# abdel-habib/mmg-clip

Hardware: AMD Instinct MI355X
Metric: image-text pairs/sec (global batch) (higher is better)
Workload: dtype bf16; 1 GPU; C2: train_binary_class_clf, ConvNeXt-tiny 1024x1024x1 + BERT-base S=77, LinearProjection 768->512, CLIPLoss, AdamW, all parameters trained; global_batch=256, per_gpu_batch=256, micro_batch=256, streams=text tower on a side stream, parallelism=dp1, loss_scope=local, text_dropout=HF training-mode dropout live (hidden 0.1, atte…

## Files before the change

### mmg-clip_amd/csrc/cnblock_mlp.hip

```cpp
#include "common.h"
#include <stdlib.h>


struct MlpFwd {
    const bf16_t* xd;
    const float* ln_w; const float* ln_b; float eps;
    const bf16_t* wt;
    const float* b1; const float* b2; const float* gamma;
    const bf16_t* res;
    bf16_t* y;
    bf16_t* hpre;
    bf16_t* xln;
    float* mean; float* rstd;
    long M; int ntiles;
    int nt;
    bf16_t* gact;
    int hkind;
};

__device__ __forceinline__ void mlp_glds16(const void* gsrc, void* lds_wave_base) {
    __builtin_amdgcn_global_load_lds((const __attribute__((address_space(1))) void*)gsrc,
                                     (__attribute__((address_space(3))) void*)lds_wave_base, 16, 0, 0);
}

template <int C> struct MlpCfg {
    static constexpr int NC = (C <= 128) ? 64 : 32;
    static constexpr int MT = (C <= 256) ? 2 : 1;
    static constexpr int WAVES = (C <= 256) ? 4 : 8;
    static constexpr int THREADS = WAVES * 64;
    static constexpr int BM = WAVES * 16 * MT;
    static constexpr int WGS = (C <= 96) ? 3 : (C <= 192 ? 2 : 1);
    static constexpr int WGS_BWD = (C <= 192) ? 2 : 1;
};

struct PackPart { const float* src; int w2_like; const float* scale; int btype; };
struct PackArgs { PackPart part[3]; int parts; bf16_t* out; int C, NC; };

__global__ __launch_bounds__(256) void mlp_pack_kernel(const PackArgs a) {
    const int C = a.C, NC = a.NC, H4 = 4 * C;
    const long per_part = (long)NC * C, per_chunk = per_part * a.parts, total = per_chunk * (H4 / NC);
    for (long e = (long)blockIdx.x * blockDim.x + threadIdx.x; e < total; e += (long)gridDim.x * blockDim.x) {
        const int j = (int)(e / per_chunk);
        long off = e - (long)j * per_chunk;
        const int pi = (int)(off / per_part);
        off -= (long)pi * per_part;
        const PackPart pp = a.part[pi];
        int n, c;
        if (!pp.btype) {
            const int kg = (int)(off / (NC * 8)), nn = (int)((off / 8) % NC), jj = (int)(off % 8);
            const int g32 = nn >> 5, tt = (nn >> 4) & 1, q = (nn >> 2) & 3, r = nn & 3;
            n = j * NC + 32 * g32 + 8 * q + 4 * tt + r; c = 8 * kg + jj;
        } else {
            const int kg = (int)(off / (C * 8)), jj = (int)(off % 8);
            const int cp = (int)((off / 8) % C);
            c = (cp & ~31) + 8 * ((cp >> 2) & 3) + 4 * ((cp >> 4) & 1) + (cp & 3);
            n = j * NC + 8 * kg + jj;
        }
        float v = pp.w2_like ? pp.src[(long)c * H4 + n] : pp.src[(long)n * C + c];
        if (pp.scale) v *= pp.scale[c];
        a.out[e] = f2bf(v);
    }
}

#ifdef MLP_PROBE
__device__ unsigned long long g_mlp_probe[8];
MMG_API int mmg_debug_mlp_probe(unsigned long long* out8, int reset) {
    if (out8 && hipMemcpyFromSymbol(out8, HIP_SYMBOL(g_mlp_probe), 64) != hipSuccess) return 1;
    unsigned long long z[8] = {0, 0, 0, 0, 0, 0, 0, 0};
    if (reset && hipMemcpyToSymbol(HIP_SYMBOL(g_mlp_probe), z, 64) != hipSuccess) return 1;
    return 0;
}
#define PROBE_T(var) const long long var = __builtin_readcyclecounter()
#define PROBE_ADD(acc, a, b) acc += (b) - (a)
#else
#define PROBE_T(var)
#define PROBE_ADD(acc, a, b)
#endif

template <int C, bool SAVE, int RW = 0>
__global__ __launch_bounds__(RW ? RW * 64 : MlpCfg<C>::THREADS, RW ? RW / 4 : MlpCfg<C>::WGS) void cnblock_mlp_fwd_kernel(const MlpFwd p) {
    constexpr bool RES = RW > 0;
    constexpr int NC = MlpCfg<C>::NC, MT = MlpCfg<C>::MT, MLP_THREADS = RES ? RW * 64 : MlpCfg<C>::THREADS;
    constexpr int MLP_BM = RES ? 16 * MT : MlpCfg<C>::BM;
    constexpr int KS1 = C / 32, CT = C / 16, NSUB = NC / 32, NCH = 4 * C / NC;
    constexpr int PART = NC * C * 2, CHUNK = 2 * PART, LOADS = CHUNK / 16 / MLP_THREADS;
    static_assert(CHUNK % (16 * MLP_THREADS) == 0, "chunk must be a whole number of 16-byte granules per thread");
    static_assert(NCH % 2 == 0, "ring parity is carried across tiles");
    static_assert(!RES || (!SAVE && NCH * CHUNK + 8 * C * 4 <= 160 * 1024), "resident form: every chunk image in LDS, nothing saved");
    extern __shared__ __attribute__((aligned(16))) char smem[];
    float* s_lnw = reinterpret_cast<float*>(smem + (RES ? NCH : 2) * CHUNK);
    float* s_lnb = s_lnw + C;
    float* s_b1 = s_lnb + C;
    float* s_b2 = s_b1 + 4 * C;
    float* s_gm = s_b2 + C;

    const int tid = threadIdx.x, lane = tid & 63;
    const int wave = RES ? __builtin_amdgcn_readfirstlane(tid >> 6) : tid >> 6;
    const int li = lane & 15, lg = lane >> 4;
    char* lds_wave = smem + (tid & ~63) * 16;
    const char* wsrc = reinterpret_cast<const char*>(p.wt) + tid * 16;

    auto stage = [&](int buf, int ch) {
        const char* s = wsrc + (size_t)ch * CHUNK;
#pragma unroll
        for (int it = 0; it < LOADS; ++it) mlp_glds16(s + it * (MLP_THREADS * 16), lds_wave + buf * CHUNK + it * (MLP_THREADS * 16));
    };
    if constexpr (RES) {
#pragma unroll
        for (int ch = 0; ch < NCH; ++ch) stage(ch, ch);
    } else if ((int)blockIdx.x < p.ntiles) stage(0, 0);
    for (int i = tid; i < C; i += MLP_THREADS) {
        s_lnw[i] = p.ln_w[i]; s_lnb[i] = p.ln_b[i]; s_b2[i] = p.b2[i]; s_gm[i] = p.gamma[i];
    }
    for (int i = tid; i < 4 * C; i += MLP_THREADS) s_b1[i] = p.b1[i];
    if constexpr (RES) asm volatile("s_waitcnt vmcnt(0)" ::: "memory");
    __syncthreads();

#ifdef MLP_PROBE
    long long pr_wait = 0, pr_g1 = 0, pr_gelu = 0, pr_g2 = 0;
#endif
    PROBE_T(pr_start);
    for (int tile = RES ? (int)blockIdx.x * RW + wave : (int)blockIdx.x; tile < p.ntiles; tile += RES ? (int)gridDim.x * RW : (int)gridDim.x) {
        const long row0 = RES ? (long)tile * MLP_BM + li : (long)tile * MLP_BM + wave * (16 * MT) + li;
        bf16x8 xf[MT][KS1];
#pragma unroll
        for (int mi = 0; mi < MT; ++mi) {
            const long row = row0 + 16 * mi;
            const long rr = row < p.M ? row : p.M - 1;
            uint4 raw[KS1];
#pragma unroll
            for (int ks = 0; ks < KS1; ++ks) raw[ks] = *reinterpret_cast<const uint4*>(p.xd + rr * C + 32 * ks + 8 * lg);
            float v[KS1][8];
            float s = 0.f;
#pragma unroll
            for (int ks = 0; ks < KS1; ++ks) {
                const unsigned w[4] = {raw[ks].x, raw[ks].y, raw[ks].z, raw[ks].w};
#pragma unroll
                for (int e = 0; e < 4; ++e) {
                    v[ks][2 * e] = bf2f_lo(w[e]); v[ks][2 * e + 1] = bf2f_hi(w[e]);
                    s += v[ks][2 * e] + v[ks][2 * e + 1];
                }
            }
            s += __shfl_xor(s, 16, 64); s += __shfl_xor(s, 32, 64);
            const float mean = s * (1.0f / C);
            float q = 0.f;
#pragma unroll
            for (int ks = 0; ks < KS1; ++ks)
#pragma unroll
                for (int e = 0; e < 8; ++e) { const float d = v[ks][e] - mean; q = fmaf(d, d, q); }
            q += __shfl_xor(q, 16, 64); q += __shfl_xor(q, 32, 64);
            const float rstd = rsqrtf(q * (1.0f / C) + p.eps);
            if (SAVE && lg == 0 && row < p.M) { p.mean[row] = mean; p.rstd[row] = rstd; }
#pragma unroll
            for (int ks = 0; ks < KS1; ++ks) {
                const f32x4 w0 = *reinterpret_cast<const f32x4*>(s_lnw + 32 * ks + 8 * lg);
                const f32x4 w1 = *reinterpret_cast<const f32x4*>(s_lnw + 32 * ks + 8 * lg + 4);
                const f32x4 c0 = *reinterpret_cast<const f32x4*>(s_lnb + 32 * ks + 8 * lg);
                const f32x4 c1 = *reinterpret_cast<const f32x4*>(s_lnb + 32 * ks + 8 * lg + 4);
                const float g[8] = {w0[0], w0[1], w0[2], w0[3], w1[0], w1[1], w1[2], w1[3]};
                const float b[8] = {c0[0], c0[1], c0[2], c0[3], c1[0], c1[1], c1[2], c1[3]};
                unsigned o[4];
#pragma unroll
                for (int e = 0; e < 4; ++e)
                    o[e] = pack2bf(fmaf((v[ks][2 * e] - mean) * rstd, g[2 * e], b[2 * e]),
                                   fmaf((v[ks][2 * e + 1] - mean) * rstd, g[2 * e + 1], b[2 * e + 1]));
                typedef __attribute__((ext_vector_type(4))) unsigned u32x4_t;
                xf[mi][ks] = __builtin_bit_cast(bf16x8, (u32x4_t{o[0], o[1], o[2], o[3]}));
                if (SAVE && p.xln && row < p.M) *reinterpret_cast<uint4*>(p.xln + row * C + 32 * ks + 8 * lg) = make_uint4(o[0], o[1], o[2], o[3]);
            }
        }

        f32x4 yacc[MT][CT];
#pragma unroll
        for (int mi = 0; mi < MT; ++mi)
#pragma unroll
            for (int ct = 0; ct < CT; ++ct) yacc[mi][ct] = f32x4{0.f, 0.f, 0.f, 0.f};

        for (int ch = 0; ch < NCH; ++ch) {
            PROBE_T(pr_a);
            if constexpr (!RES) {
                asm volatile("s_waitcnt vmcnt(0)" ::: "memory");
                __builtin_amdgcn_s_barrier();
            }
            PROBE_T(pr_b);
            PROBE_ADD(pr_wait, pr_a, pr_b);
            if constexpr (!RES) {
                if (ch + 1 < NCH) stage((ch + 1) & 1, ch + 1);
                else if (tile + (int)gridDim.x < p.ntiles) stage(0, 0);
            }
            const char* wb = smem + (RES ? ch : (ch & 1)) * CHUNK;
#pragma unroll
            for (int sub = 0; sub < NSUB; ++sub) {
#if defined(MLP_PROBE) && MLP_PROBE >= 2
                PROBE_T(pr_c);
#endif
                const int n0 = ch * NC + sub * 32 + 8 * lg;
                const f32x4 bia0 = *reinterpret_cast<const f32x4*>(s_b1 + n0);
                const f32x4 bia1 = *reinterpret_cast<const f32x4*>(s_b1 + n0 + 4);
                f32x4 hacc[MT][2];
#pragma unroll
                for (int mi = 0; mi < MT; ++mi) { hacc[mi][0] = bia0; hacc[mi][1] = bia1; }
#pragma unroll
                for (int ks = 0; ks < KS1; ++ks) {
#pragma unroll
                    for (int tt = 0; tt < 2; ++tt) {
                        const bf16x8 wf = *reinterpret_cast<const bf16x8*>(wb + (((4 * ks + lg) * NC + (2 * sub + tt) * 16 + li) << 4));
#pragma unroll
                        for (int mi = 0; mi < MT; ++mi)
                            hacc[mi][tt] = __builtin_amdgcn_mfma_f32_16x16x32_bf16(wf, xf[mi][ks], hacc[mi][tt], 0, 0, 0);
                    }
                }
#if defined(MLP_PROBE) && MLP_PROBE >= 2
                asm volatile("" : "+v"(hacc[0][0]), "+v"(hacc[MT - 1][1]));
                PROBE_T(pr_d);
                PROBE_ADD(pr_g1, pr_c, pr_d);
#endif
                bf16x8 gf[MT];
#pragma unroll
                for (int mi = 0; mi < MT; ++mi) {
                    const f32x4 h0 = hacc[mi][0], h1 = hacc[mi][1];
                    if (SAVE) {
                        const long row = row0 + 16 * mi;
                        if (row < p.M) {
                            if (p.hkind)
                                store16_stream(p.hpre + row * (4 * C) + n0,
                                               make_uint4(pack2bf(gelu_bf16_grad_poly(h0[0]), gelu_bf16_grad_poly(h0[1])), pack2bf(gelu_bf16_grad_poly(h0[2]), gelu_bf16_grad_poly(h0[3])),
                                                          pack2bf(gelu_bf16_grad_poly(h1[0]), gelu_bf16_grad_poly(h1[1])), pack2bf(gelu_bf16_grad_poly(h1[2]), gelu_bf16_grad_poly(h1[3]))), p.nt);
                            else
                                store16_stream(p.hpre + row * (4 * C) + n0,
                                               make_uint4(pack2bf(h0[0], h0[1]), pack2bf(h0[2], h0[3]), pack2bf(h1[0], h1[1]), pack2bf(h1[2], h1[3])), p.nt);
                        }
                    }
                    typedef __attribute__((ext_vector_type(4))) unsigned u32x4_t;
                    gf[mi] = __builtin_bit_cast(bf16x8, (u32x4_t{pack2bf(gelu_bf16(h0[0]), gelu_bf16(h0[1])), pack2bf(gelu_bf16(h0[2]), gelu_bf16(h0[3])),
                                                                 pack2bf(gelu_bf16(h1[0]), gelu_bf16(h1[1])), pack2bf(gelu_bf16(h1[2]), gelu_bf16(h1[3]))}));
                    if (SAVE) {
                        const long row = row0 + 16 * mi;
                        if (p.gact && row < p.M) {
                            const u32x4_t gw = __builtin_bit_cast(u32x4_t, gf[mi]);
                            store16_stream(p.gact + row * (4 * C) + n0, make_uint4(gw[0], gw[1], gw[2], gw[3]), p.nt);
                        }
                    }
                }
#if defined(MLP_PROBE) && MLP_PROBE >= 2
                asm volatile("" : "+v"(gf[0]), "+v"(gf[MT - 1]));
                PROBE_T(pr_e);
                PROBE_ADD(pr_gelu, pr_d, pr_e);
#endif
#pragma unroll
                for (int ct = 0; ct < CT; ++ct) {
                    const bf16x8 wf = *reinterpret_cast<const bf16x8*>(wb + PART + (((4 * sub + lg) * C + ct * 16 + li) << 4));
#pragma unroll
                    for (int mi = 0; mi < MT; ++mi)
                        yacc[mi][ct] = __builtin_amdgcn_mfma_f32_16x16x32_bf16(wf, gf[mi], yacc[mi][ct], 0, 0, 0);
                }
#if defined(MLP_PROBE) && MLP_PROBE >= 2
                asm volatile("" : "+v"(yacc[0][0]), "+v"(yacc[MT - 1][CT - 1]));
                PROBE_T(pr_f);
                PROBE_ADD(pr_g2, pr_e, pr_f);
#endif
            }
        }

        int lane_e;
        asm volatile("v_mbcnt_lo_u32_b32 %0, -1, 0\n\tv_mbcnt_hi_u32_b32 %0, -1, %0" : "=v"(lane_e));
        const int lg_e = lane_e >> 4;
#pragma unroll
        for (int mi = 0; mi < MT; ++mi) {
            const long row = row0 + 16 * mi;
            if (row < p.M) {
                uint4 rv[CT / 2];
#pragma unroll
                for (int j = 0; j < CT / 2; ++j) rv[j] = *reinterpret_cast<const uint4*>(p.res + row * C + 32 * j + 8 * lg_e);
#pragma unroll
                for (int j = 0; j < CT / 2; ++j) {
                    const int c8 = 32 * j + 8 * lg_e;
                    const unsigned rw[4] = {rv[j].x, rv[j].y, rv[j].z, rv[j].w};
                    unsigned o[4];
#pragma unroll
                    for (int h = 0; h < 2; ++h) {
                        const f32x4 b2 = *reinterpret_cast<const f32x4*>(s_b2 + c8 + 4 * h);
                        const f32x4 gm = *reinterpret_cast<const f32x4*>(s_gm + c8 + 4 * h);
                        const f32x4 a = yacc[mi][2 * j + h];
                        o[2 * h] = pack2bf(fmaf(gm[0], a[0] + b2[0], bf2f_lo(rw[2 * h])), fmaf(gm[1], a[1] + b2[1], bf2f_hi(rw[2 * h])));
                        o[2 * h + 1] = pack2bf(fmaf(gm[2], a[2] + b2[2], bf2f_lo(rw[2 * h + 1])), fmaf(gm[3], a[3] + b2[3], bf2f_hi(rw[2 * h + 1])));
                    }
                    *reinterpret_cast<uint4*>(p.y + row * C + c8) = make_uint4(o[0], o[1], o[2], o[3]);
                }
            }
        }
    }
#ifdef MLP_PROBE
    PROBE_T(pr_end);
    if (lane == 0) {
        atomicAdd(&g_mlp_probe[0], (unsigned long long)(pr_end - pr_start)); atomicAdd(&g_mlp_probe[1], (unsigned long long)pr_wait);
        atomicAdd(&g_mlp_probe[2], (unsigned long long)pr_g1); atomicAdd(&g_mlp_probe[3], (unsigned long long)pr_gelu);
        atomicAdd(&g_mlp_probe[4], (unsigned long long)pr_g2); atomicAdd(&g_mlp_probe[5], 1ull);
    }
#endif
}

struct MlpBwd {
    const bf16_t* dy;
    const bf16_t* xd;
    const float* ln_w; const float* ln_b; float eps;
    const bf16_t* wt;
    const float* b1;
    bf16_t* dh; bf16_t* g;
    bf16_t* xln; bf16_t* dxln;
    float* mean; float* rstd;
    const bf16_t* hpre;
    float* ln_dw; float* ln_db;
    long M; int ntiles;
    int nt;
};

__device__ __forceinline__ float row16_sum(float v) {
    v += __int_as_float(__builtin_amdgcn_mov_dpp(__float_as_int(v), 0xB1, 0xf, 0xf, true));
    v += __int_as_float(__builtin_amdgcn_mov_dpp(__float_as_int(v), 0x4E, 0xf, 0xf, true));
    v += __int_as_float(__builtin_amdgcn_mov_dpp(__float_as_int(v), 0x141, 0xf, 0xf, true));
    v += __int_as_float(__builtin_amdgcn_mov_dpp(__float_as_int(v), 0x140, 0xf, 0xf, true));
    return v;
}

template <int C, bool RECOMP, bool LNB>
__global__ __launch_bounds__(MlpCfg<C>::THREADS, MlpCfg<C>::WGS_BWD) void cnblock_mlp_bwd_kernel(const MlpBwd p) {
    constexpr int NC = MlpCfg<C>::NC, MT = MlpCfg<C>::MT, MLP_THREADS = MlpCfg<C>::THREADS, MLP_BM = MlpCfg<C>::BM;
    constexpr int KS1 = C / 32, CT = C / 16, NSUB = NC / 32, NCH = 4 * C / NC;
    constexpr int NPART = RECOMP ? 3 : 2, P_W2 = RECOMP ? 1 : 0, P_W1T = RECOMP ? 2 : 1;
    constexpr int PART = NC * C * 2, CHUNK = NPART * PART, LOADS = CHUNK / 16 / MLP_THREADS;
    static_assert(CHUNK % (16 * MLP_THREADS) == 0, "chunk must be a whole number of 16-byte granules per thread");
    static_assert(NCH % 2 == 0, "ring parity is carried across tiles");
    typedef __attribute__((ext_vector_type(4))) unsigned u32x4_t;
    extern __shared__ __attribute__((aligned(16))) char smem[];
    float* s_lnw = reinterpret_cast<float*>(smem + 2 * CHUNK);
    float* s_lnb = s_lnw + C;
    float* s_b1 = s_lnb + C;
    float* s_dg = s_b1 + 4 * C;
    float* s_db = s_dg + C;

    const int tid = threadIdx.x, lane = tid & 63;
    const int wave = __builtin_amdgcn_readfirstlane(tid >> 6);
    const int li = lane & 15, lg = lane >> 4;
    char* lds_wave = smem + (tid & ~63) * 16;
    const __amdgpu_buffer_rsrc_t rs_w = __builtin_amdgcn_make_buffer_rsrc((void*)p.wt, 0, NCH * CHUNK, 0x27000);
    const int toff = tid * 16;
    auto stage = [&](int buf, int ch) {
#pragma unroll
        for (int it = 0; it < LOADS; ++it)
            __builtin_amdgcn_raw_ptr_buffer_load_lds(rs_w, (__attribute__((address_space(3))) void*)(lds_wave + buf * CHUNK + it * (MLP_THREADS * 16)), 16, toff,
                                                 ch * CHUNK + it * (MLP_THREADS * 16), 0, 0);
    };
    const int soff = (li * (4 * C) + 8 * lg) * 2;
    if ((int)blockIdx.x < p.ntiles) stage(0, 0);
    for (int i = tid; i < C; i += MLP_THREADS) { s_lnw[i] = p.ln_w[i]; s_lnb[i] = p.ln_b[i]; s_dg[i] = 0.f; s_db[i] = 0.f; }
    for (int i = tid; i < 4 * C; i += MLP_THREADS) s_b1[i] = p.b1[i];
    __syncthreads();

    for (int tile = blockIdx.x; tile < p.ntiles; tile += gridDim.x) {
        const long row0 = (long)tile * MLP_BM + wave * (16 * MT) + li;
        const long wrow0 = (long)tile * MLP_BM + wave * (16 * MT);
        const long wrows = p.M - wrow0 < 0 ? 0 : (p.M - wrow0 < 16 * MT ? p.M - wrow0 : 16 * MT);
        const __amdgpu_buffer_rsrc_t rs_g = __builtin_amdgcn_make_buffer_rsrc((void*)(p.g + wrow0 * (4 * C)), 0, (int)(wrows * (4 * C) * 2), 0x27000);
        const __amdgpu_buffer_rsrc_t rs_dh = __builtin_amdgcn_make_buffer_rsrc((void*)(p.dh + wrow0 * (4 * C)), 0, (int)(wrows * (4 * C) * 2), 0x27000);
        bf16x8 xf[RECOMP ? MT : 1][RECOMP ? KS1 : 1], dyf[MT][KS1];
        float row_mean[MT], row_rstd[MT];
        int lane_t;
        asm volatile("v_mbcnt_lo_u32_b32 %0, -1, 0\n\tv_mbcnt_hi_u32_b32 %0, -1, %0" : "=v"(lane_t));
        const int lg_t = lane_t >> 4;
#pragma unroll
        for (int mi = 0; mi < MT; ++mi) {
            const long row = row0 + 16 * mi;
            const long rr = row < p.M ? row : p.M - 1;
            uint4 raw[KS1];
#pragma unroll
            for (int ks = 0; ks < KS1; ++ks) {
                raw[ks] = *reinterpret_cast<const uint4*>(p.xd + rr * C + 32 * ks + 8 * lg_t);
                const uint4 dv = *reinterpret_cast<const uint4*>(p.dy + rr * C + 32 * ks + 8 * lg_t);
                dyf[mi][ks] = __builtin_bit_cast(bf16x8, (u32x4_t{dv.x, dv.y, dv.z, dv.w}));
            }
            float v[KS1][8];
            float s = 0.f;
#pragma unroll
            for (int ks = 0; ks < KS1; ++ks) {
                const unsigned w[4] = {raw[ks].x, raw[ks].y, raw[ks].z, raw[ks].w};
#pragma unroll
                for (int e = 0; e < 4; ++e) {
                    v[ks][2 * e] = bf2f_lo(w[e]); v[ks][2 * e + 1] = bf2f_hi(w[e]);
                    s += v[ks][2 * e] + v[ks][2 * e + 1];
                }
            }
            s += __shfl_xor(s, 16, 64); s += __shfl_xor(s, 32, 64);
            const float mean = s * (1.0f / C);
            float q = 0.f;
#pragma unroll
            for (int ks = 0; ks < KS1; ++ks)
#pragma unroll
                for (int e = 0; e < 8; ++e) { const float d = v[ks][e] - mean; q = fmaf(d, d, q); }
            q += __shfl_xor(q, 16, 64); q += __shfl_xor(q, 32, 64);
            const float rstd = rsqrtf(q * (1.0f / C) + p.eps);
            if (lg == 0 && row < p.M) { p.mean[row] = mean; p.rstd[row] = rstd; }
            row_mean[mi] = mean; row_rstd[mi] = rstd;
#pragma unroll
            for (int ks = 0; ks < KS1; ++ks) {
                const f32x4 w0 = *reinterpret_cast<const f32x4*>(s_lnw + 32 * ks + 8 * lg);
                const f32x4 w1 = *reinterpret_cast<const f32x4*>(s_lnw + 32 * ks + 8 * lg + 4);
                const f32x4 c0 = *reinterpret_cast<const f32x4*>(s_lnb + 32 * ks + 8 * lg);
                const f32x4 c1 = *reinterpret_cast<const f32x4*>(s_lnb + 32 * ks + 8 * lg + 4);
                const float g[8] = {w0[0], w0[1], w0[2], w0[3], w1[0], w1[1], w1[2], w1[3]};
                const float b[8] = {c0[0], c0[1], c0[2], c0[3], c1[0], c1[1], c1[2], c1[3]};
                unsigned o[4];
#pragma unroll
                for (int e = 0; e < 4; ++e)
                    o[e] = pack2bf(fmaf((v[ks][2 * e] - mean) * rstd, g[2 * e], b[2 * e]),
                                   fmaf((v[ks][2 * e + 1] - mean) * rstd, g[2 * e + 1], b[2 * e + 1]));
                if (RECOMP) xf[RECOMP ? mi : 0][RECOMP ? ks : 0] = __builtin_bit_cast(bf16x8, (u32x4_t{o[0], o[1], o[2], o[3]}));
                if (row < p.M) *reinterpret_cast<uint4*>(p.xln + row * C + 32 * ks + 8 * lg_t) = make_uint4(o[0], o[1], o[2], o[3]);
            }
        }

        f32x4 dxacc[MT][CT];
#pragma unroll
        for (int mi = 0; mi < MT; ++mi)
#pragma unroll
            for (int ct = 0; ct < CT; ++ct) dxacc[mi][ct] = f32x4{0.f, 0.f, 0.f, 0.f};

        for (int ch = 0; ch < NCH; ++ch) {
            constexpr int NST_CH = 2 * MT * NSUB;
            if (RECOMP && ch > 0) asm volatile("s_waitcnt vmcnt(%0)" ::"n"(NST_CH) : "memory");
            else asm volatile("s_waitcnt vmcnt(0)" ::: "memory");
            __builtin_amdgcn_s_barrier();
            if (ch + 1 < NCH) stage((ch + 1) & 1, ch + 1);
            else if (tile + (int)gridDim.x < p.ntiles) stage(0, 0);
            const char* wb = smem + (ch & 1) * CHUNK;
#pragma unroll
            for (int sub = 0; sub < NSUB; ++sub) {
                const int n0 = ch * NC + sub * 32 + 8 * lg;
                const f32x4 bia0 = *reinterpret_cast<const f32x4*>(s_b1 + n0);
                const f32x4 bia1 = *reinterpret_cast<const f32x4*>(s_b1 + n0 + 4);
                f32x4 hacc[MT][2], gacc[MT][2];
#pragma unroll
                for (int mi = 0; mi < MT; ++mi) {
                    if (RECOMP) {
                        hacc[mi][0] = bia0; hacc[mi][1] = bia1;
                    } else {
                        const long row = row0 + 16 * mi;
                        const long rr = row < p.M ? row : p.M - 1;
                        const uint4 u = *reinterpret_cast<const uint4*>(p.hpre + rr * (4 * C) + n0);
                        hacc[mi][0] = f32x4{bf2f_lo(u.x), bf2f_hi(u.x), bf2f_lo(u.y), bf2f_hi(u.y)};
                        hacc[mi][1] = f32x4{bf2f_lo(u.z), bf2f_hi(u.z), bf2f_lo(u.w), bf2f_hi(u.w)};
                    }
                    gacc[mi][0] = f32x4{0.f, 0.f, 0.f, 0.f}; gacc[mi][1] = f32x4{0.f, 0.f, 0.f, 0.f};
                }
#pragma unroll
                for (int ks = 0; ks < KS1; ++ks) {
#pragma unroll
                    for (int tt = 0; tt < 2; ++tt) {
                        const int off = ((4 * ks + lg) * NC + (2 * sub + tt) * 16 + li) << 4;
                        const bf16x8 w2f = *reinterpret_cast<const bf16x8*>(wb + P_W2 * PART + off);
                        if (RECOMP) {
                            const bf16x8 w1f = *reinterpret_cast<const bf16x8*>(wb + off);
#pragma unroll
                            for (int mi = 0; mi < MT; ++mi)
                                hacc[mi][tt] = __builtin_amdgcn_mfma_f32_16x16x32_bf16(w1f, xf[RECOMP ? mi : 0][RECOMP ? ks : 0], hacc[mi][tt], 0, 0, 0);
                        }
#pragma unroll
                        for (int mi = 0; mi < MT; ++mi)
                            gacc[mi][tt] = __builtin_amdgcn_mfma_f32_16x16x32_bf16(w2f, dyf[mi][ks], gacc[mi][tt], 0, 0, 0);
                    }
                }
                bf16x8 dhf[MT];
#pragma unroll
                for (int mi = 0; mi < MT; ++mi) {
                    unsigned gp[4], dp[4];
#pragma unroll
                    for (int tt = 0; tt < 2; ++tt) {
                        float a[4], d[4];
#pragma unroll
                        for (int e = 0; e < 4; ++e) {
                            float dg;
                            gelu_bf16_both(hacc[mi][tt][e], a[e], dg);
                            d[e] = gacc[mi][tt][e] * dg;
                        }
                        gp[2 * tt] = pack2bf(a[0], a[1]); gp[2 * tt + 1] = pack2bf(a[2], a[3]);
                        dp[2 * tt] = pack2bf(d[0], d[1]); dp[2 * tt + 1] = pack2bf(d[2], d[3]);
                    }
                    dhf[mi] = __builtin_bit_cast(bf16x8, (u32x4_t{dp[0], dp[1], dp[2], dp[3]}));
                    {
                        const int vo = soff + mi * (16 * 4 * C * 2), so = (ch * NC + sub * 32) * 2;
                        if (p.nt) {
                            __builtin_amdgcn_raw_buffer_store_b128(u32x4_t{gp[0], gp[1], gp[2], gp[3]}, rs_g, vo, so, 2);
                            __builtin_amdgcn_raw_buffer_store_b128(u32x4_t{dp[0], dp[1], dp[2], dp[3]}, rs_dh, vo, so, 2);
                        } else {
                            __builtin_amdgcn_raw_buffer_store_b128(u32x4_t{gp[0], gp[1], gp[2], gp[3]}, rs_g, vo, so, 0);
                            __builtin_amdgcn_raw_buffer_store_b128(u32x4_t{dp[0], dp[1], dp[2], dp[3]}, rs_dh, vo, so, 0);
                        }
                    }
                }
#pragma unroll
                for (int ct = 0; ct < CT; ++ct) {
                    const bf16x8 wf = *reinterpret_cast<const bf16x8*>(wb + P_W1T * PART + (((4 * sub + lg) * C + ct * 16 + li) << 4));
#pragma unroll
                    for (int mi = 0; mi < MT; ++mi)
                        dxacc[mi][ct] = __builtin_amdgcn_mfma_f32_16x16x32_bf16(wf, dhf[mi], dxacc[mi][ct], 0, 0, 0);
                }
            }
        }
        int lane_x;
        asm volatile("v_mbcnt_lo_u32_b32 %0, -1, 0\n\tv_mbcnt_hi_u32_b32 %0, -1, %0" : "=v"(lane_x));
        const int lg_x = lane_x >> 4;
        if (!LNB) {
#pragma unroll
            for (int mi = 0; mi < MT; ++mi) {
                const long row = row0 + 16 * mi;
                if (row < p.M) {
#pragma unroll
                    for (int j = 0; j < CT / 2; ++j) {
                        const f32x4 a = dxacc[mi][2 * j], b = dxacc[mi][2 * j + 1];
                        *reinterpret_cast<uint4*>(p.dxln + row * C + 32 * j + 8 * lg_x) =
                            make_uint4(pack2bf(a[0], a[1]), pack2bf(a[2], a[3]), pack2bf(b[0], b[1]), pack2bf(b[2], b[3]));
                    }
                }
            }
        } else {
            uint2 xv[MT][CT];
            float m1[MT], m2[MT];
#pragma unroll
            for (int mi = 0; mi < MT; ++mi) {
                const long row = row0 + 16 * mi;
                const long rr = row < p.M ? row : p.M - 1;
#pragma unroll
                for (int ct = 0; ct < CT; ++ct) xv[mi][ct] = *reinterpret_cast<const uint2*>(p.xd + rr * C + 32 * (ct >> 1) + 8 * lg_x + 4 * (ct & 1));
                float s1 = 0.f, s2 = 0.f;
#pragma unroll
                for (int ct = 0; ct < CT; ++ct) {
                    const f32x4 gm = *reinterpret_cast<const f32x4*>(s_lnw + 32 * (ct >> 1) + 8 * lg + 4 * (ct & 1));
                    const float x[4] = {bf2f_lo(xv[mi][ct].x), bf2f_hi(xv[mi][ct].x), bf2f_lo(xv[mi][ct].y), bf2f_hi(xv[mi][ct].y)};
#pragma unroll
                    for (int r = 0; r < 4; ++r) {
                        const float xh = (x[r] - row_mean[mi]) * row_rstd[mi];
                        const float gg = dxacc[mi][ct][r] * gm[r];
                        s1 += gg; s2 = fmaf(gg, xh, s2);
                    }
                }
                s1 += __shfl_xor(s1, 16, 64); s1 += __shfl_xor(s1, 32, 64);
                s2 += __shfl_xor(s2, 16, 64); s2 += __shfl_xor(s2, 32, 64);
                m1[mi] = s1 * (1.0f / C); m2[mi] = s2 * (1.0f / C);
            }
#pragma unroll
            for (int ct = 0; ct < CT; ++ct) {
                const int cc = 32 * (ct >> 1) + 8 * lg_x + 4 * (ct & 1);
                const f32x4 gm = *reinterpret_cast<const f32x4*>(s_lnw + cc);
                float cg[4] = {0.f, 0.f, 0.f, 0.f}, cb[4] = {0.f, 0.f, 0.f, 0.f};
#pragma unroll
                for (int mi = 0; mi < MT; ++mi) {
                    const long row = row0 + 16 * mi;
                    const bool ok = row < p.M;
                    const float x[4] = {bf2f_lo(xv[mi][ct].x), bf2f_hi(xv[mi][ct].x), bf2f_lo(xv[mi][ct].y), bf2f_hi(xv[mi][ct].y)};
                    float o[4];
#pragma unroll
                    for (int r = 0; r < 4; ++r) {
                        const float xh = (x[r] - row_mean[mi]) * row_rstd[mi];
                        const float dv = ok ? dxacc[mi][ct][r] : 0.f;
                        o[r] = row_rstd[mi] * (fmaf(-xh, m2[mi], dv * gm[r]) - m1[mi]);
                        cg[r] = fmaf(dv, xh, cg[r]); cb[r] += dv;
                    }
                    if (ok) *reinterpret_cast<uint2*>(p.dxln + row * C + cc) = make_uint2(pack2bf(o[0], o[1]), pack2bf(o[2], o[3]));
                }
#pragma unroll
                for (int r = 0; r < 4; ++r) {
                    const float tg = row16_sum(cg[r]), tb = row16_sum(cb[r]);
                    if (li == 0) { atomicAdd(s_dg + cc + r, tg); atomicAdd(s_db + cc + r, tb); }
                }
            }
        }
    }
    if (LNB) {
        __syncthreads();
        for (int i = tid; i < C; i += MLP_THREADS) { atomicAdd(p.ln_dw + i, s_dg[i]); atomicAdd(p.ln_db + i, s_db[i]); }
    }
}

#define MLP_FWD_RES_DEFAULT 12
static int mlp_cu_count() { return mmg_cu_count_cached(); }

static int mlp_nt_store(long M, int C, bool backward) {
    const char* e = getenv("MMG_MLP_NT_STORE");
    if (e) return atoi(e) != 0;
    return backward && C >= 128 && (size_t)M * 4 * C * 2 >= ((size_t)256 << 20);
}

template <int C, bool RECOMP>
static int launch_mlp_bwd(MlpBwd p, hipStream_t stream) {
    typedef MlpCfg<C> Cfg;
    p.nt = mlp_nt_store(p.M, C, true);
    const size_t lds = 2 * ((RECOMP ? 3 : 2) * Cfg::NC * C * 2) + (size_t)8 * C * sizeof(float);
    p.ntiles = (int)((p.M + Cfg::BM - 1) / Cfg::BM);
    const int cap = Cfg::WGS_BWD * mlp_cu_count();
    const int grid = p.ntiles < cap ? p.ntiles : cap;
    MMG_NOTE_KERNEL("cnblock_mlp_bwd_kernel<%d, %s, %s>", C, RECOMP ? "true" : "false", p.ln_dw ? "true" : "false");
    if (p.ln_dw) {
        mmg_allow_lds(cnblock_mlp_bwd_kernel<C, RECOMP, true>, lds);
        hipLaunchKernelGGL((cnblock_mlp_bwd_kernel<C, RECOMP, true>), dim3(grid), dim3(Cfg::THREADS), lds, stream, p);
    } else {
        mmg_allow_lds(cnblock_mlp_bwd_kernel<C, RECOMP, false>, lds);
        hipLaunchKernelGGL((cnblock_mlp_bwd_kernel<C, RECOMP, false>), dim3(grid), dim3(Cfg::THREADS), lds, stream, p);
    }
    MMG_LAUNCH_CHECK("mmg_cnblock_mlp_bwd");
    return 0;
}

template <int C>
static int launch_mlp_fwd(MlpFwd p, hipStream_t stream) {
    typedef MlpCfg<C> Cfg;
    p.nt = p.hpre ? mlp_nt_store(p.M, C, false) : 0;
    const size_t lds = 2 * (2 * Cfg::NC * C * 2) + (size_t)8 * C * sizeof(float);
    p.ntiles = (int)((p.M + Cfg::BM - 1) / Cfg::BM);
    const int cap = Cfg::WGS * mlp_cu_count();
    const int grid = p.ntiles < cap ? p.ntiles : cap;
    if constexpr (C == 96) {
        const char* e = getenv("MMG_MLP_FWD_RES");
        const int rw = e ? atoi(e) : MLP_FWD_RES_DEFAULT;
        if (!p.hpre && (rw == 8 || rw == 12)) {
            const size_t ldsr = (size_t)(4 * C / Cfg::NC) * (2 * Cfg::NC * C * 2) + (size_t)8 * C * sizeof(float);
            p.ntiles = (int)((p.M + 16 * Cfg::MT - 1) / (16 * Cfg::MT));
            const int cus = mlp_cu_count();
            const int gridr = (p.ntiles + rw - 1) / rw < cus ? (p.ntiles + rw - 1) / rw : cus;
            MMG_NOTE_KERNEL("cnblock_mlp_fwd_kernel<%d, false, %d>", C, rw);
            if (rw == 12) {
                mmg_allow_lds(cnblock_mlp_fwd_kernel<C, false, 12>, ldsr);
                hipLaunchKernelGGL((cnblock_mlp_fwd_kernel<C, false, 12>), dim3(gridr), dim3(768), ldsr, stream, p);
            } else {
                mmg_allow_lds(cnblock_mlp_fwd_kernel<C, false, 8>, ldsr);
                hipLaunchKernelGGL((cnblock_mlp_fwd_kernel<C, false, 8>), dim3(gridr), dim3(512), ldsr, stream, p);
            }
            MMG_LAUNCH_CHECK("mmg_cnblock_mlp_fwd");
            return 0;
        }
    }
    MMG_NOTE_KERNEL("cnblock_mlp_fwd_kernel<%d, %s>", C, p.hpre ? "true" : "false");
    if (p.hpre) {
        mmg_allow_lds(cnblock_mlp_fwd_kernel<C, true>, lds);
        hipLaunchKernelGGL((cnblock_mlp_fwd_kernel<C, true>), dim3(grid), dim3(Cfg::THREADS), lds, stream, p);
    } else {
        mmg_allow_lds(cnblock_mlp_fwd_kernel<C, false>, lds);
        hipLaunchKernelGGL((cnblock_mlp_fwd_kernel<C, false>), dim3(grid), dim3(Cfg::THREADS), lds, stream, p);
    }
    MMG_LAUNCH_CHECK("mmg_cnblock_mlp_fwd");
    return 0;
}

static bool mlp_supported(int C) { return C == 96 || C == 128 || C == 192 || C == 256 || C == 384 || C == 512; }

MMG_API long long mmg_cnblock_packed_elems(int C, int backward) {
    if (!mlp_supported(C)) return 0;
    return (long long)(backward == 1 ? 3 : 2) * 4 * C * C;
}

MMG_API int mmg_cnblock_pack_weights(const float* w1, const float* w2, const float* gamma, void* packed, int C, int backward,
                                     hipStream_t stream) {
    MMG_CHECK_ARG(w1 && w2 && packed, "mmg_cnblock_pack_weights: null pointer");
    MMG_CHECK_ARG(mlp_supported(C), "mmg_cnblock_pack_weights: C=%d not in {96,128,192,256,384,512}", C);
    MMG_CHECK_ARG(backward >= 0 && backward <= 2, "mmg_cnblock_pack_weights: backward=%d not in {0,1,2}", backward);
    MMG_CHECK_ARG(!backward || gamma, "mmg_cnblock_pack_weights: the backward image needs the layer scale");
    PackArgs a{};
    a.out = (bf16_t*)packed; a.C = C; a.NC = C <= 128 ? 64 : 32;
    a.part[0] = PackPart{w1, 0, nullptr, 0};
    if (!backward) {
        a.parts = 2;
        a.part[1] = PackPart{w2, 1, nullptr, 1};
    } else if (backward == 1) {
        a.parts = 3;
        a.part[1] = PackPart{w2, 1, gamma, 0};
        a.part[2] = PackPart{w1, 0, nullptr, 1};
    } else {
        a.parts = 2;
        a.part[0] = PackPart{w2, 1, gamma, 0};
        a.part[1] = PackPart{w1, 0, nullptr, 1};
    }
    hipLaunchKernelGGL(mlp_pack_kernel, dim3(256), dim3(256), 0, stream, a);
    MMG_LAUNCH_CHECK("mmg_cnblock_pack_weights");
    return 0;
}

MMG_API int mmg_cnblock_mlp_fwd(const void* xd, const float* ln_w, const float* ln_b, float eps, const void* packed,
                                const float* b1, const float* b2, const float* gamma, const void* residual, void* y,
                                void* hpre, void* xln, void* gact, float* mean, float* rstd, int hpre_kind, long long M, int C, hipStream_t stream) {
    MMG_CHECK_ARG(xd && ln_w && ln_b && packed && b1 && b2 && gamma && residual && y, "mmg_cnblock_mlp_fwd: null pointer");
    MMG_CHECK_ARG(mlp_supported(C), "mmg_cnblock_mlp_fwd: C=%d not in {96,128,192,256,384,512}", C);
    MMG_CHECK_ARG(M > 0 && M < (1LL << 36), "mmg_cnblock_mlp_fwd: bad M=%lld", M);
    MMG_CHECK_ARG((mean == nullptr) == (hpre == nullptr) && (rstd == nullptr) == (hpre == nullptr),
                  "mmg_cnblock_mlp_fwd: hpre, mean and rstd are saved together or not at all");
    MMG_CHECK_ARG(!xln || hpre, "mmg_cnblock_mlp_fwd: xln is saved next to hpre only");
    MMG_CHECK_ARG(!gact || hpre, "mmg_cnblock_mlp_fwd: gact is saved next to hpre only");
    MlpFwd p{(const bf16_t*)xd, ln_w, ln_b, eps, (const bf16_t*)packed, b1, b2, gamma, (const bf16_t*)residual, (bf16_t*)y,
             (bf16_t*)hpre, (bf16_t*)xln, mean, rstd, (long)M, 0, 0, (bf16_t*)gact, hpre_kind};
    MMG_CHECK_ARG(hpre_kind == 0 || (hpre_kind == 1 && hpre && gact), "mmg_cnblock_mlp_fwd: hpre_kind=%d (1 = GELU' in place of the pre-activation) needs hpre and gact", hpre_kind);
    switch (C) {
        case 96: return launch_mlp_fwd<96>(p, stream);
        case 128: return launch_mlp_fwd<128>(p, stream);
        case 192: return launch_mlp_fwd<192>(p, stream);
        case 256: return launch_mlp_fwd<256>(p, stream);
        case 384: return launch_mlp_fwd<384>(p, stream);
        default: return launch_mlp_fwd<512>(p, stream);
    }
}

MMG_API int mmg_cnblock_mlp_bwd_supported(int C) { return (C == 96 || C == 128 || C == 192) ? 1 : (C == 384 ? 2 : 0); }

MMG_API int mmg_cnblock_mlp_bwd(const void* dy, const void* xd, const float* ln_w, const float* ln_b, float eps,
                                const void* packed_bwd, const float* b1, const void* hpre, void* dh, void* g, void* xln,
                                void* dxln, float* mean, float* rstd, float* ln_dw, float* ln_db, long long M, int C,
                                hipStream_t stream) {
    MMG_CHECK_ARG(dy && xd && ln_w && ln_b && packed_bwd && b1 && dh && g && xln && dxln && mean && rstd,
                  "mmg_cnblock_mlp_bwd: null pointer");
    const int mode = mmg_cnblock_mlp_bwd_supported(C);
    MMG_CHECK_ARG(mode != 0, "mmg_cnblock_mlp_bwd: C=%d not in {96,128,192,384}", C);
    MMG_CHECK_ARG((mode == 2) == (hpre != nullptr), "mmg_cnblock_mlp_bwd: hpre is required for C=384 and unused otherwise (C=%d)", C);
    MMG_CHECK_ARG(M > 0 && M < (1LL << 36), "mmg_cnblock_mlp_bwd: bad M=%lld", M);
    MMG_CHECK_ARG((ln_dw == nullptr) == (ln_db == nullptr), "mmg_cnblock_mlp_bwd: ln_dw and ln_db go together");
    MlpBwd p{(const bf16_t*)dy, (const bf16_t*)xd, ln_w, ln_b, eps, (const bf16_t*)packed_bwd, b1, (bf16_t*)dh, (bf16_t*)g,
             (bf16_t*)xln, (bf16_t*)dxln, mean, rstd, (const bf16_t*)hpre, ln_dw, ln_db, (long)M, 0, 0};
    switch (C) {
        case 96: return launch_mlp_bwd<96, true>(p, stream);
        case 128: return launch_mlp_bwd<128, true>(p, stream);
        case 192: return launch_mlp_bwd<192, true>(p, stream);
        default: return launch_mlp_bwd<384, false>(p, stream);
    }
}
```

Before: 889.4 image-text pairs/sec.

## Add pipelined C=384 ConvNeXt MLP forward form with buffer stores and fragment ring

Adds forward variants for the C=384 ConvNeXt block MLP kernel, chosen by an environment variable that defaults to form 2. Form 2 runs 4 waves with two m-tiles each, stages weights through buffer-resource loads into LDS, and prefetches weight fragments through a six-deep register ring with scheduling barriers so LDS reads overlap the MFMAs. The saving forms fix which activations are saved as template parameters, write hpre and gact through bounds-checked buffer stores, and wait on a counted vmcnt so outstanding stores do not stall the weight pipeline. The cost is more register pressure, changed occupancy at C=384, and more template instantiations.

```diff
diff --git a/mmg-clip_amd/csrc/cnblock_mlp.hip b/mmg-clip_amd/csrc/cnblock_mlp.hip
--- a/mmg-clip_amd/csrc/cnblock_mlp.hip
+++ b/mmg-clip_amd/csrc/cnblock_mlp.hip
@@ -31,6 +31,15 @@
     static constexpr int BM = WAVES * 16 * MT;
     static constexpr int WGS = (C <= 96) ? 3 : (C <= 192 ? 2 : 1);
     static constexpr int WGS_BWD = (C <= 192) ? 2 : 1;
+};
+
+template <int C, int FORM> struct MlpFwdCfg {
+    static_assert(FORM == 0 || C == 384, "forms 1 and 2 exist at C = 384 only");
+    static constexpr int MT = (FORM == 2) ? 2 : MlpCfg<C>::MT;
+    static constexpr int WAVES = (FORM == 2) ? 4 : MlpCfg<C>::WAVES;
+    static constexpr int THREADS = WAVES * 64;
+    static constexpr int BM = WAVES * 16 * MT;
+    static constexpr int WGS = MlpCfg<C>::WGS;
 };
 
 struct PackPart { const float* src; int w2_like; const float* scale; int btype; };
@@ -77,11 +86,14 @@
 #define PROBE_ADD(acc, a, b)
 #endif
 
-template <int C, bool SAVE, int RW = 0>
-__global__ __launch_bounds__(RW ? RW * 64 : MlpCfg<C>::THREADS, RW ? RW / 4 : MlpCfg<C>::WGS) void cnblock_mlp_fwd_kernel(const MlpFwd p) {
+template <int C, bool SAVE, int RW = 0, int FORM = 0, int SK = 0>
+__global__ __launch_bounds__((RW ? RW * 64 : MlpFwdCfg<C, FORM>::THREADS), (RW ? RW / 4 : MlpFwdCfg<C, FORM>::WGS)) void cnblock_mlp_fwd_kernel(const MlpFwd p) {
     constexpr bool RES = RW > 0;
-    constexpr int NC = MlpCfg<C>::NC, MT = MlpCfg<C>::MT, MLP_THREADS = RES ? RW * 64 : MlpCfg<C>::THREADS;
-    constexpr int MLP_BM = RES ? 16 * MT : MlpCfg<C>::BM;
+    constexpr bool CNT = SAVE && FORM > 0;
+    static_assert((SAVE && FORM > 0) || SK == 0, "the save set is a template parameter of the counted saving form only");
+    static_assert(!(SK & 1) || (SK & 2), "GELU' in `hpre` goes with `gact`");
+    constexpr int NC = MlpCfg<C>::NC, MT = MlpFwdCfg<C, FORM>::MT, MLP_THREADS = RES ? RW * 64 : MlpFwdCfg<C, FORM>::THREADS;
+    constexpr int MLP_BM = RES ? 16 * MT : MlpFwdCfg<C, FORM>::BM;
     constexpr int KS1 = C / 32, CT = C / 16, NSUB = NC / 32, NCH = 4 * C / NC;
     constexpr int PART = NC * C * 2, CHUNK = 2 * PART, LOADS = CHUNK / 16 / MLP_THREADS;
     static_assert(CHUNK % (16 * MLP_THREADS) == 0, "chunk must be a whole number of 16-byte granules per thread");
@@ -95,15 +107,22 @@
     float* s_gm = s_b2 + C;
 
     const int tid = threadIdx.x, lane = tid & 63;
-    const int wave = RES ? __builtin_amdgcn_readfirstlane(tid >> 6) : tid >> 6;
+    const int wave = (RES || CNT) ? __builtin_amdgcn_readfirstlane(tid >> 6) : tid >> 6;
     const int li = lane & 15, lg = lane >> 4;
     char* lds_wave = smem + (tid & ~63) * 16;
     const char* wsrc = reinterpret_cast<const char*>(p.wt) + tid * 16;
 
+    const __amdgpu_buffer_rsrc_t rs_w = __builtin_amdgcn_make_buffer_rsrc((void*)p.wt, 0, NCH * CHUNK, 0x27000);
     auto stage = [&](int buf, int ch) {
         const char* s = wsrc + (size_t)ch * CHUNK;
 #pragma unroll
-        for (int it = 0; it < LOADS; ++it) mlp_glds16(s + it * (MLP_THREADS * 16), lds_wave + buf * CHUNK + it * (MLP_THREADS * 16));
+        for (int it = 0; it < LOADS; ++it) {
+            if constexpr (FORM == 2)
+                __builtin_amdgcn_raw_ptr_buffer_load_lds(rs_w, (__attribute__((address_space(3))) void*)(lds_wave + buf * CHUNK + it * (MLP_THREADS * 16)), 16, tid * 16,
+                                                     ch * CHUNK + it * (MLP_THREADS * 16), 0, 0);
+            else
+                mlp_glds16(s + it * (MLP_THREADS * 16), lds_wave + buf * CHUNK + it * (MLP_THREADS * 16));
+        }
     };
     if constexpr (RES) {
 #pragma unroll
@@ -122,6 +141,15 @@
     PROBE_T(pr_start);
     for (int tile = RES ? (int)blockIdx.x * RW + wave : (int)blockIdx.x; tile < p.ntiles; tile += RES ? (int)gridDim.x * RW : (int)gridDim.x) {
         const long row0 = RES ? (long)tile * MLP_BM + li : (long)tile * MLP_BM + wave * (16 * MT) + li;
+        const bool sv_hk = CNT ? (SK & 1) != 0 : p.hkind != 0;
+        const bool sv_gact = CNT ? (SK & 2) != 0 : p.gact != nullptr;
+        const bool sv_xln = CNT ? (SK & 4) != 0 : p.xln != nullptr;
+        typedef __attribute__((ext_vector_type(4))) unsigned u32x4_t;
+        const int soff = (li * (4 * C) + 8 * lg) * 2;
+        const long wrow0 = (long)tile * MLP_BM + wave * (16 * MT);
+        const long wrows = p.M - wrow0 < 0 ? 0 : (p.M - wrow0 < 16 * MT ? p.M - wrow0 : 16 * MT);
+        const __amdgpu_buffer_rsrc_t rs_h = __builtin_amdgcn_make_buffer_rsrc((void*)(p.hpre + wrow0 * (4 * C)), 0, (int)(wrows * (4 * C) * 2), 0x27000);
+        const __amdgpu_buffer_rsrc_t rs_g = __builtin_amdgcn_make_buffer_rsrc((void*)(p.gact + wrow0 * (4 * C)), 0, (int)(wrows * (4 * C) * 2), 0x27000);
         bf16x8 xf[MT][KS1];
 #pragma unroll
         for (int mi = 0; mi < MT; ++mi) {
@@ -164,9 +192,8 @@
                 for (int e = 0; e < 4; ++e)
                     o[e] = pack2bf(fmaf((v[ks][2 * e] - mean) * rstd, g[2 * e], b[2 * e]),
                                    fmaf((v[ks][2 * e + 1] - mean) * rstd, g[2 * e + 1], b[2 * e + 1]));
-                typedef __attribute__((ext_vector_type(4))) unsigned u32x4_t;
                 xf[mi][ks] = __builtin_bit_cast(bf16x8, (u32x4_t{o[0], o[1], o[2], o[3]}));
-                if (SAVE && p.xln && row < p.M) *reinterpret_cast<uint4*>(p.xln + row * C + 32 * ks + 8 * lg) = make_uint4(o[0], o[1], o[2], o[3]);
+                if (SAVE && sv_xln && row < p.M) *reinterpret_cast<uint4*>(p.xln + row * C + 32 * ks + 8 * lg) = make_uint4(o[0], o[1], o[2], o[3]);
             }
         }
 
@@ -179,7 +206,9 @@
         for (int ch = 0; ch < NCH; ++ch) {
             PROBE_T(pr_a);
             if constexpr (!RES) {
-                asm volatile("s_waitcnt vmcnt(0)" ::: "memory");
+                constexpr int NST_CH = MT * NSUB * ((SK & 2) ? 2 : 1);
+                if (CNT && ch > 0) asm volatile("s_waitcnt vmcnt(%0)" ::"n"(NST_CH) : "memory");
+                else asm volatile("s_waitcnt vmcnt(0)" ::: "memory");
                 __builtin_amdgcn_s_barrier();
             }
             PROBE_T(pr_b);
@@ -187,6 +216,7 @@
             if constexpr (!RES) {
                 if (ch + 1 < NCH) stage((ch + 1) & 1, ch + 1);
                 else if (tile + (int)gridDim.x < p.ntiles) stage(0, 0);
+                if constexpr (CNT) __builtin_amdgcn_sched_barrier(0);
             }
             const char* wb = smem + (RES ? ch : (ch & 1)) * CHUNK;
 #pragma unroll
@@ -200,14 +230,36 @@
                 f32x4 hacc[MT][2];
 #pragma unroll
                 for (int mi = 0; mi < MT; ++mi) { hacc[mi][0] = bia0; hacc[mi][1] = bia1; }
-#pragma unroll
-                for (int ks = 0; ks < KS1; ++ks) {
-#pragma unroll
-                    for (int tt = 0; tt < 2; ++tt) {
-                        const bf16x8 wf = *reinterpret_cast<const bf16x8*>(wb + (((4 * ks + lg) * NC + (2 * sub + tt) * 16 + li) << 4));
+                constexpr int RING = FORM == 2 ? 6 : 1, NFRAG = 2 * KS1 + CT;
+                bf16x8 ring[RING];
+                auto frag = [&](int f) {
+                    const int off = f < 2 * KS1 ? (((4 * (f >> 1) + lg) * NC + (2 * sub + (f & 1)) * 16 + li) << 4)
+                                                : PART + (((4 * sub + lg) * C + (f - 2 * KS1) * 16 + li) << 4);
+                    return *reinterpret_cast<const bf16x8*>(wb + off);
+                };
+                if constexpr (FORM == 2) {
+#pragma unroll
+                    for (int f = 0; f < RING; ++f) ring[f] = frag(f);
+#pragma unroll
+                    for (int f = 0; f < 2 * KS1; ++f) {
+                        __builtin_amdgcn_sched_barrier(0);
+                        const bf16x8 wf = ring[f % RING];
 #pragma unroll
                         for (int mi = 0; mi < MT; ++mi)
-                            hacc[mi][tt] = __builtin_amdgcn_mfma_f32_16x16x32_bf16(wf, xf[mi][ks], hacc[mi][tt], 0, 0, 0);
+                            hacc[mi][f & 1] = __builtin_amdgcn_mfma_f32_16x16x32_bf16(wf, xf[mi][f >> 1], hacc[mi][f & 1], 0, 0, 0);
+                        ring[f % RING] = frag(f + RING);
+                    }
+                    __builtin_amdgcn_sched_barrier(0);
+                } else {
+#pragma unroll
+                    for (int ks = 0; ks < KS1; ++ks) {
+#pragma unroll
+                        for (int tt = 0; tt < 2; ++tt) {
+                            const bf16x8 wf = frag(2 * ks + tt);
+#pragma unroll
+                            for (int mi = 0; mi < MT; ++mi)
+                                hacc[mi][tt] = __builtin_amdgcn_mfma_f32_16x16x32_bf16(wf, xf[mi][ks], hacc[mi][tt], 0, 0, 0);
+                        }
                     }
                 }
 #if defined(MLP_PROBE) && MLP_PROBE >= 2
@@ -219,10 +271,15 @@
 #pragma unroll
                 for (int mi = 0; mi < MT; ++mi) {
                     const f32x4 h0 = hacc[mi][0], h1 = hacc[mi][1];
-                    if (SAVE) {
+                    if constexpr (CNT) {
+                        const u32x4_t hw = (SK & 1) ? u32x4_t{pack2bf(gelu_bf16_grad_poly(h0[0]), gelu_bf16_grad_poly(h0[1])), pack2bf(gelu_bf16_grad_poly(h0[2]), gelu_bf16_grad_poly(h0[3])),
+                                                              pack2bf(gelu_bf16_grad_poly(h1[0]), gelu_bf16_grad_poly(h1[1])), pack2bf(gelu_bf16_grad_poly(h1[2]), gelu_bf16_grad_poly(h1[3]))}
+                                                    : u32x4_t{pack2bf(h0[0], h0[1]), pack2bf(h0[2], h0[3]), pack2bf(h1[0], h1[1]), pack2bf(h1[2], h1[3])};
+                        __builtin_amdgcn_raw_buffer_store_b128(hw, rs_h, soff + mi * (16 * 4 * C * 2) + (ch * NC + sub * 32) * 2, 0, 0);
+                    } else if (SAVE) {
                         const long row = row0 + 16 * mi;
                         if (row < p.M) {
-                            if (p.hkind)
+                            if (sv_hk)
                                 store16_stream(p.hpre + row * (4 * C) + n0,
                                                make_uint4(pack2bf(gelu_bf16_grad_poly(h0[0]), gelu_bf16_grad_poly(h0[1])), pack2bf(gelu_bf16_grad_poly(h0[2]), gelu_bf16_grad_poly(h0[3])),
                                                           pack2bf(gelu_bf16_grad_poly(h1[0]), gelu_bf16_grad_poly(h1[1])), pack2bf(gelu_bf16_grad_poly(h1[2]), gelu_bf16_grad_poly(h1[3]))), p.nt);
@@ -231,12 +288,14 @@
                                                make_uint4(pack2bf(h0[0], h0[1]), pack2bf(h0[2], h0[3]), pack2bf(h1[0], h1[1]), pack2bf(h1[2], h1[3])), p.nt);
                         }
                     }
-                    typedef __attribute__((ext_vector_type(4))) unsigned u32x4_t;
                     gf[mi] = __builtin_bit_cast(bf16x8, (u32x4_t{pack2bf(gelu_bf16(h0[0]), gelu_bf16(h0[1])), pack2bf(gelu_bf16(h0[2]), gelu_bf16(h0[3])),
                                                                  pack2bf(gelu_bf16(h1[0]), gelu_bf16(h1[1])), pack2bf(gelu_bf16(h1[2]), gelu_bf16(h1[3]))}));
-                    if (SAVE) {
+                    if constexpr (CNT) {
+                        if constexpr ((SK & 2) != 0)
+                            __builtin_amdgcn_raw_buffer_store_b128(__builtin_bit_cast(u32x4_t, gf[mi]), rs_g, soff + mi * (16 * 4 * C * 2) + (ch * NC + sub * 32) * 2, 0, 0);
+                    } else if (SAVE) {
                         const long row = row0 + 16 * mi;
-                        if (p.gact && row < p.M) {
+                        if (sv_gact && row < p.M) {
                             const u32x4_t gw = __builtin_bit_cast(u32x4_t, gf[mi]);
                             store16_stream(p.gact + row * (4 * C) + n0, make_uint4(gw[0], gw[1], gw[2], gw[3]), p.nt);
                         }
@@ -247,12 +306,25 @@
                 PROBE_T(pr_e);
                 PROBE_ADD(pr_gelu, pr_d, pr_e);
 #endif
-#pragma unroll
-                for (int ct = 0; ct < CT; ++ct) {
-                    const bf16x8 wf = *reinterpret_cast<const bf16x8*>(wb + PART + (((4 * sub + lg) * C + ct * 16 + li) << 4));
-#pragma unroll
-                    for (int mi = 0; mi < MT; ++mi)
-                        yacc[mi][ct] = __builtin_amdgcn_mfma_f32_16x16x32_bf16(wf, gf[mi], yacc[mi][ct], 0, 0, 0);
+                if constexpr (FORM == 2) {
+#pragma unroll
+                    for (int f = 2 * KS1; f < NFRAG; ++f) {
+                        __builtin_amdgcn_sched_barrier(0);
+                        const bf16x8 wf = ring[f % RING];
+#pragma unroll
+                        for (int mi = 0; mi < MT; ++mi)
+                            yacc[mi][f - 2 * KS1] = __builtin_amdgcn_mfma_f32_16x16x32_bf16(wf, gf[mi], yacc[mi][f - 2 * KS1], 0, 0, 0);
+                        if (f + RING < NFRAG) ring[f % RING] = frag(f + RING);
+                    }
+                    __builtin_amdgcn_sched_barrier(0);
+                } else {
+#pragma unroll
+                    for (int ct = 0; ct < CT; ++ct) {
+                        const bf16x8 wf = frag(2 * KS1 + ct);
+#pragma unroll
+                        for (int mi = 0; mi < MT; ++mi)
+                            yacc[mi][ct] = __builtin_amdgcn_mfma_f32_16x16x32_bf16(wf, gf[mi], yacc[mi][ct], 0, 0, 0);
+                    }
                 }
 #if defined(MLP_PROBE) && MLP_PROBE >= 2
                 asm volatile("" : "+v"(yacc[0][0]), "+v"(yacc[MT - 1][CT - 1]));
@@ -610,15 +682,39 @@
     return 0;
 }
 
-template <int C>
-static int launch_mlp_fwd(MlpFwd p, hipStream_t stream) {
-    typedef MlpCfg<C> Cfg;
-    p.nt = p.hpre ? mlp_nt_store(p.M, C, false) : 0;
-    const size_t lds = 2 * (2 * Cfg::NC * C * 2) + (size_t)8 * C * sizeof(float);
+#define MLP_FWD_384_DEFAULT 2
+
+template <int C, int FORM, bool SAVE, int SK>
+static int mlp_fwd_go(MlpFwd p, hipStream_t stream) {
+    typedef MlpFwdCfg<C, FORM> Cfg;
+    p.nt = (SAVE && FORM == 0) ? mlp_nt_store(p.M, C, false) : 0;
+    const size_t lds = 2 * (2 * MlpCfg<C>::NC * C * 2) + (size_t)8 * C * sizeof(float);
     p.ntiles = (int)((p.M + Cfg::BM - 1) / Cfg::BM);
     const int cap = Cfg::WGS * mlp_cu_count();
     const int grid = p.ntiles < cap ? p.ntiles : cap;
+    mmg_allow_lds(cnblock_mlp_fwd_kernel<C, SAVE, 0, FORM, SK>, lds);
+    hipLaunchKernelGGL((cnblock_mlp_fwd_kernel<C, SAVE, 0, FORM, SK>), dim3(grid), dim3(Cfg::THREADS), lds, stream, p);
+    MMG_LAUNCH_CHECK("mmg_cnblock_mlp_fwd");
+    return 0;
+}
+
+template <int C, int FORM>
+static int mlp_fwd_save(const MlpFwd& p, hipStream_t stream) {
+    switch ((p.hkind ? 1 : 0) | (p.gact ? 2 : 0) | (p.xln ? 4 : 0)) {
+        case 0: return mlp_fwd_go<C, FORM, true, 0>(p, stream);
+        case 2: return mlp_fwd_go<C, FORM, true, 2>(p, stream);
+        case 3: return mlp_fwd_go<C, FORM, true, 3>(p, stream);
+        case 4: return mlp_fwd_go<C, FORM, true, 4>(p, stream);
+        case 6: return mlp_fwd_go<C, FORM, true, 6>(p, stream);
+        case 7: return mlp_fwd_go<C, FORM, true, 7>(p, stream);
+        default: mmg_set_error("mmg_cnblock_mlp_fwd: GELU' in hpre needs gact"); return 1;
+    }
+}
+
+template <int C>
+static int launch_mlp_fwd(MlpFwd p, hipStream_t stream) {
     if constexpr (C == 96) {
+        typedef MlpCfg<C> Cfg;
         const char* e = getenv("MMG_MLP_FWD_RES");
         const int rw = e ? atoi(e) : MLP_FWD_RES_DEFAULT;
         if (!p.hpre && (rw == 8 || rw == 12)) {
@@ -639,15 +735,14 @@
         }
     }
     MMG_NOTE_KERNEL("cnblock_mlp_fwd_kernel<%d, %s>", C, p.hpre ? "true" : "false");
-    if (p.hpre) {
-        mmg_allow_lds(cnblock_mlp_fwd_kernel<C, true>, lds);
-        hipLaunchKernelGGL((cnblock_mlp_fwd_kernel<C, true>), dim3(grid), dim3(Cfg::THREADS), lds, stream, p);
-    } else {
-        mmg_allow_lds(cnblock_mlp_fwd_kernel<C, false>, lds);
-        hipLaunchKernelGGL((cnblock_mlp_fwd_kernel<C, false>), dim3(grid), dim3(Cfg::THREADS), lds, stream, p);
-    }
-    MMG_LAUNCH_CHECK("mmg_cnblock_mlp_fwd");
-    return 0;
+    if constexpr (C == 384) {
+        const char* e = getenv("MMG_MLP_FWD_384");
+        const int form = e ? atoi(e) : MLP_FWD_384_DEFAULT;
+        MMG_CHECK_ARG(form >= 0 && form <= 2, "mmg_cnblock_mlp_fwd: MMG_MLP_FWD_384=%d not in {0,1,2}", form);
+        if (form == 2) return p.hpre ? mlp_fwd_save<C, 2>(p, stream) : mlp_fwd_go<C, 2, false, 0>(p, stream);
+        if (form == 1 && p.hpre) return mlp_fwd_save<C, 1>(p, stream);
+    }
+    return p.hpre ? mlp_fwd_go<C, 0, true, 0>(p, stream) : mlp_fwd_go<C, 0, false, 0>(p, stream);
 }
 
 static bool mlp_supported(int C) { return C == 96 || C == 128 || C == 192 || C == 256 || C == 384 || C == 512; }
```

Result: no change. 897.2 image-text pairs/sec, median of 6 (+0.9%).
